# Yan-Xia/Text2Loc

Hardware: AMD Instinct MI355X
Metric: coarse-retrieval queries/sec over 11k-cell DB, embed_dim=256; top-1/3/5 recall parity (higher is better)
Workload: dtype f16; 1 GPU; KITTI360Pose-sized val DB: N=11259 cells x D=256 resident in HBM, Q=4096 precomputed text embeddings per step, top-10 (float64-exact ids); n_cells=11259, embed_dim=256, top_k=10, parallelism=single-gpu, layout=one resident DB, two launches per step (scan, re-rank)

## Files before the change

### text2loc_amd/csrc/capi.hip

```cpp
#include <limits.h>
#include <string.h>

#include "t2l_internal.h"

namespace t2l {

int fail(t2l_ctx* ctx, int code, const std::string& msg) {
  if (ctx) ctx->err = msg;
  return code;
}

void event_begin(t2l_ctx* ctx, const char* name, hipStream_t s) {
  if (!ctx->profile_events) return;
  EventRing& e = ctx->events[name];
  if (e.a.empty()) {
    e.a.resize(kEventRing);
    e.b.resize(kEventRing);
    for (int i = 0; i < kEventRing; ++i) {
      (void)hipEventCreate(&e.a[i]);
      (void)hipEventCreate(&e.b[i]);
    }
  }
  e.open = (e.calls++ % ctx->profile_events) == 0;
  if (e.open) (void)hipEventRecord(e.a[e.head], s);
// ... 558 lines not shown
    if (!ctx->search_auto) {
      ctx->escalated = false;
      ctx->heavy = false;
      ctx->all_exact = false;
      ctx->merge_live = true;
      ctx->stat_seen = ctx->stat_seq;
    }
  } else if (!strcmp(name, "search_heavy")) {
    ctx->heavy = value != 0;
  } else if (!strcmp(name, "search_small")) {
    ctx->search_small = value != 0;
  } else if (!strcmp(name, "search_small_wgs")) {
    if (value < 0 || value > 256) return fail(ctx, T2L_EINVAL, "search_small_wgs: 0 (default by query count: 128 or 192) .. 256 workgroups per slice");
    ctx->search_small_wgs = (int)value;
  } else if (!strcmp(name, "search_xcd_qgroups")) {
    if (value != 1 && value != 2 && value != 4 && value != 8) return fail(ctx, T2L_EINVAL, "search_xcd_qgroups must be 1, 2, 4 or 8");
    ctx->xcd_qgroups = (int)value;
  } else if (!strcmp(name, "text_train_bf16")) {
    if (value != 1 && value != 2)
      return fail(ctx, T2L_EINVAL, "text_train_bf16: 2 (default: split-bf16, the f32-class arithmetic) or 1 (bf16 operands); the f32-MFMA "
                                   "form (0) was removed in round 5 — it measured slower than PyTorch's f32 step");
    ctx->text_train_bf16 = (int)value;
  } else if (!strcmp(name, "encoder_two_cells")) {
    ctx->encoder_two_cells = value != 0;
  } else if (!strcmp(name, "search_merge_lists")) {
    if (value != 0 && value != 1 && value != 2) return fail(ctx, T2L_EINVAL, "search_merge_lists: 0 (plain lists), 1 (merged records), 2 (default: by report card)");
    ctx->search_merge = (int)value;
    ctx->merge_live = true;
  } else if (!strcmp(name, "search_wide_repair")) {
    if (value < 0 || value > 1024) return fail(ctx, T2L_EINVAL, "search_wide_repair: 0 (off) .. 1024 rows");
    ctx->wide_repair = (int)value;
  } else if (!strcmp(name, "search_tile_sel")) {
    ctx->search_tile_sel = value != 0;
  } else if (!strcmp(name, "search_pair_ll")) {
    if (value != 5 && value != 6) return fail(ctx, T2L_EINVAL, "search_pair_ll must be 5 or 6");
    ctx->pair_ll = (int)value;
  } else if (!strcmp(name, "train_gemm_block")) {
    if (value != 0 && value != 32 && value != 64) return fail(ctx, T2L_EINVAL, "train_gemm_block must be 0 (auto), 32 or 64");
    ctx->train_gemm_block = (int)value;
  } else if (!strcmp(name, "train_bf16")) {
    if (value != 0 && value != 1 && value != 2) return fail(ctx, T2L_EINVAL, "train_bf16: 0 (f32 MFMA), 1 (bf16 operands) or 2 (split-bf16, three products)");
    ctx->train_bf16 = (int)value;
  } else if (!strcmp(name, "train_keep_adam_state")) {
    ctx->train_keep_adam = value != 0;
  } else if (!strcmp(name, "profile_rerank")) {
    ctx->profile_rerank = value != 0;
  } else if (!strcmp(name, "stats_reset")) {
    for (auto& kv : ctx->events) {
      kv.second.count = 0;
      kv.second.calls = 0;
      kv.second.open = false;
    }
    ctx->span_read = ctx->busy_read = ctx->span_seq;
  } else if (!strcmp(name, "search_lanes")) {
    if (value < 1 || value > t2l_ctx::kMaxLanes) return fail(ctx, T2L_EINVAL, "search_lanes must be 1..4");
    T2L_HIP(ctx, hipDeviceSynchronize());
    for (auto& L : ctx->lanes) L.pending = false;
    ctx->n_lanes = (int)value;
  } else if (!strcmp(name, "stream_min_rows")) {
    ctx->stream_min_rows = (int)value;
  } else if (!strcmp(name, "pointnet_pyg_self_loops")) {
    ctx->pn_self_loops = value != 0;
  } else if (!strcmp(name, "profile_events")) {
    if (value < 0) return fail(ctx, T2L_EINVAL, "profile_events must be >= 0");
    ctx->profile_events = (int)value;
    for (auto& kv : ctx->events) kv.second.calls = 0;
// ... 10 lines not shown
  const bool busy = !strcmp(name, "search_scan_busy");
  if (busy || !strcmp(name, "search_scan_span")) {
    unsigned& cursor = busy ? ctx->busy_read : ctx->span_read;
    if (!ctx->scan_span || ctx->span_seq == cursor) return T2L_OK;
    T2L_HIP(ctx, hipDeviceSynchronize());
    std::vector<unsigned long long> h((size_t)2 * kSpanWgs * kSpanRing);
    T2L_HIP(ctx, hipMemcpy(h.data(), ctx->scan_span, sizeof(unsigned long long) * h.size(), hipMemcpyDeviceToHost));
    const unsigned first = ctx->span_seq - cursor > (unsigned)kSpanRing ? ctx->span_seq - kSpanRing + 1 : cursor + 1;
    double sum = 0.0;
    int n = 0;
    const unsigned long long tmask = (1ull << 40) - 1;
    for (unsigned q = first; q <= ctx->span_seq; ++q) {
      const unsigned long long* e = &h[(size_t)2 * kSpanWgs * (q % kSpanRing)];
      const unsigned grid = ctx->span_grid[q % kSpanRing];
      if (!grid) continue;
      unsigned long long t_min = ~0ull, t_max = 0, total = 0;
      bool ok = true;
      for (unsigned w = 0; w < grid && ok; ++w) {
        const unsigned long long a = e[2 * w], b = e[2 * w + 1];
        ok = (a >> 40) == (q & 0xFFFFFFu) && (b >> 40) == (q & 0xFFFFFFu);
        t_min = std::min(t_min, a & tmask);
        t_max = std::max(t_max, b & tmask);
        total += ((b & tmask) - (a & tmask)) & tmask;
      }
      if (!ok) continue;
      sum += (busy ? (double)total / grid : (double)((t_max - t_min) & tmask)) * 1e-5;
      ++n;
    }
    cursor = ctx->span_seq;
    if (n) *out_avg_ms = (float)(sum / n);
    *out_count = n;
    return T2L_OK;
  }
  auto it = ctx->events.find(name);
  if (it == ctx->events.end() || it->second.count == 0) return T2L_OK;
  EventRing& e = it->second;
  double sum = 0.0;
  for (int i = 0; i < e.count; ++i) {
    const int slot = ((e.head - 1 - i) % kEventRing + kEventRing) % kEventRing;
    T2L_HIP(ctx, hipEventSynchronize(e.b[slot]));
    float ms = 0.f;
    T2L_HIP(ctx, hipEventElapsedTime(&ms, e.a[slot], e.b[slot]));
    sum += ms;
  }
  *out_avg_ms = (float)(sum / e.count);
  *out_count = e.count;
  e.count = 0;
  return T2L_OK;
}

}
```

### text2loc_amd/csrc/search.hip

```cpp
#include <float.h>
#include <limits.h>

#include <type_traits>

#include "t2l_internal.h"
#include "search_dev.h"

namespace t2l {

__device__ __forceinline__ void reset_counts(int32_t* fb_count, int32_t* fb_prev, int zero_counts, int tid) {
  if (zero_counts && tid < 16) {
    fb_count[64 + tid] = fb_prev[tid];
    fb_prev[tid] = 0;
  }
  if (!zero_counts && tid == 0) {
    fb_count[12] += fb_count[4];
    fb_count[4] = fb_count[6] = 0;
  }
}


__global__ __launch_bounds__(256) void split_db_kernel(const float* __restrict__ db, uint4* __restrict__ out, int rows) {
  const int gid = blockIdx.x * 256 + threadIdx.x;
  const int row = gid >> 5, c = gid & 31;
// ... 228 lines not shown
  }
  asm volatile("s_waitcnt vmcnt(0)" ::: "memory");

  {
    const int row0 = (sp + (nt - 1) * nsplit) * kTileRows + 4 * half;
    const int code0 = (nt - 1) << 4;
    const bool odd = nt & 1;
#pragma unroll
    for (int r = 0; r < 16; ++r) {
      const bool ok = row0 + (r & 3) + 8 * (r >> 2) < n_rows;
      const float s0 = odd ? accA0[r] : accB0[r], s1 = odd ? accA1[r] : accB1[r];
      ins_key<LL>(w.ls0, ok ? make_key(s0, mask, code0 + r) : T2L_NEG_INF);
      ins_key<LL>(w.ls1, ok ? make_key(s1, mask, code0 + r) : T2L_NEG_INF);
    }
  }
  const int part = 2 * sp + half, parts = 2 * nsplit;
  if (qrow0 < Q) {
    float4* out = reinterpret_cast<float4*>(cand + ((size_t)qrow0 * parts + part) * LL);
#pragma unroll
    for (int i = 0; i < LL / 4; ++i) out[i] = make_float4(w.ls0[4 * i], w.ls0[4 * i + 1], w.ls0[4 * i + 2], w.ls0[4 * i + 3]);
  }
  if (qrow1 < Q) {
    float4* out = reinterpret_cast<float4*>(cand + ((size_t)qrow1 * parts + part) * LL);
#pragma unroll
    for (int i = 0; i < LL / 4; ++i) out[i] = make_float4(w.ls1[4 * i], w.ls1[4 * i + 1], w.ls1[4 * i + 2], w.ls1[4 * i + 3]);
  }
}

template <int CTRL>
__device__ __forceinline__ float dpp_f(float v) {
  return __uint_as_float((unsigned)__builtin_amdgcn_update_dpp(0, (int)__float_as_uint(v), CTRL, 0xF, 0xF, true));
}

struct RerankArgs {
  const float* db;
  const float* q;
  int Q, K, parts, code_bits;
  const float* cand;
  int row_offset;
  float eps_rel;
  const float* db_norm_max;
  int half_mode;
  int32_t* out_idx;
  double* out_score;
  int32_t* flags;
  int32_t* fb_count;
  float eps_rel_probe, pinf;
  int n_rows, defer, stat_mode;
  int32_t* host_stat;
  int seq, wide_cap;
  int rec6;
};

constexpr int kMergedLL = 8;
#ifndef T2L_SEL_RD
#define T2L_SEL_RD 2
#endif
template <int LL, int NS, bool MERGE = false, int SEL = 0>
__global__ __launch_bounds__(512, 1) void scanp_kernel(const uint4* __restrict__ dbt, int n_rows, int n_tiles, int code_bits,
                                                       const float* __restrict__ q, int Q, int nsplit,
                                                       float* __restrict__ cand, int32_t* __restrict__ fb_count, int32_t* __restrict__ fb_prev,
                                                       int zero_counts, float pinf, unsigned long long* __restrict__ span,
                                                       unsigned span_seq, int xcd_qgroups) {
  static_assert(NS == 4, "the step loop below is unrolled for a ring of 4 slots");
  static_assert(!MERGE || LL == 6, "the in-workgroup list merge is written for lists of 6");
  static_assert(!SEL || MERGE, "the tile-local selection's dropped-bound leaves through the merged record's bound");
  extern __shared__ __attribute__((aligned(16))) float smem[];
  constexpr int kSlotBytes = 2 * kHalfTileBytes;
  constexpr unsigned kExchange = 2 * kSlotBytes;
  const int tid = threadIdx.x, lane = tid & 63;
  const int half = lane >> 5, col = lane & 31;
  int sp = blockIdx.x % nsplit, qb = blockIdx.x / nsplit;
  if (xcd_qgroups > 1) {
    const int GQ = xcd_qgroups, GS = 8 / GQ, nqb = gridDim.x / nsplit;
    const int x = blockIdx.x & 7, j = blockIdx.x >> 3, per = nqb / GQ;
    qb = (j % per) * GQ + x % GQ;
    sp = (j / per) * GS + x / GQ;
  }
  const int uwave = uniform_wave_id();
  const int quad = uwave >> 2, wq = uwave & 3;
  const int vn = 2 * nsplit, vs = sp + quad * nsplit;
  const int nt = vs < n_tiles ? (n_tiles - vs + vn - 1) / vn : 0;
  const int steps = sp < n_tiles ? (n_tiles - sp + vn - 1) / vn : 0;
  constexpr int kCS = MERGE ? 2 : 0;
// ... 411 lines not shown
      const int b = __float_as_int(key), src = b & 3;
      return key_row(__int_as_float(b >> 2), 2 * (part + (src >> 1) * parts) + (src & 1), 2 * parts, code_bits, strided_rows);
    } else {
      return key_row(key, part, parts >> 1, code_bits, strided_rows);
    }
  };
  const float* __restrict__ cand = a.cand;
  const float eps_rel = a.eps_rel, eps_rel_probe = a.eps_rel_probe, pinf = a.pinf;
  const float* __restrict__ db_norm_max = a.db_norm_max;
  int32_t* __restrict__ out_idx = a.out_idx;
  double* __restrict__ out_score = a.out_score;
  int32_t* __restrict__ flags = a.flags;
  int32_t* __restrict__ fb_count = a.fb_count;
  const int n_rows = a.n_rows, defer = a.defer, wide_cap = a.wide_cap;

  float lst[LL];
  {
    const float* mine = cand + ((size_t)qid * parts + min(lane, parts - 1)) * LL;
    if constexpr (MG) {
      const float4 v0 = reinterpret_cast<const float4*>(mine)[0], v1 = reinterpret_cast<const float4*>(mine)[1];
      lst[0] = v0.x; lst[1] = v0.y; lst[2] = v0.z; lst[3] = v0.w;
      lst[4] = v1.x; lst[5] = v1.y; lst[6] = v1.z; lst[7] = v1.w;
    } else if constexpr (LL % 2 == 0) {
#pragma unroll
      for (int i = 0; i < LL / 2; ++i) {
        const float2 v = reinterpret_cast<const float2*>(mine)[i];
        lst[2 * i] = v.x;
        lst[2 * i + 1] = v.y;
      }
    } else {
#pragma unroll
      for (int i = 0; i < LL; ++i) lst[i] = mine[i];
    }
    if (lane >= parts) {
#pragma unroll
      for (int i = 0; i < LL; ++i) lst[i] = T2L_NEG_INF;
    }
  }
  const float lane_floor = lst[LL - 1];
  if constexpr (MG) lst[LL - 1] = T2L_NEG_INF;
  float b1 = T2L_NEG_INF;
  if constexpr (MG) {
    if (a.rec6) {
      b1 = lst[LL - 2];
      lst[LL - 2] = T2L_NEG_INF;
    }
  }
  const float floor_max = wave_max_f32(fmaxf(lane_floor, b1), pinf);
  const int seg = lane & 15;
  double qd[16];
  float q_absmax = 0.f;
  {
    const float4* qp = reinterpret_cast<const float4*>(q + (size_t)qid * kD) + seg;
#pragma unroll
    for (int i = 0; i < 4; ++i) {
      const float4 v = qp[16 * i];
      qd[4 * i] = (double)v.x;
      qd[4 * i + 1] = (double)v.y;
      qd[4 * i + 2] = (double)v.z;
      qd[4 * i + 3] = (double)v.w;
      q_absmax = fmaxf(fmaxf(fmaxf(q_absmax, fabsf(v.x)), fabsf(v.y)), fmaxf(fabsf(v.z), fabsf(v.w)));
    }
  }

  float my_key = T2L_NEG_INF;
  int my_part = 0;
  auto merge_round = [&](int r) {
    const float bk = wave_max_f32(lst[0], pinf);
    const unsigned long long who = __ballot(lst[0] == bk);
    const int bl = __ffsll((long long)who) - 1;
    if (lane == r) {
      my_key = bk;
      my_part = bl;
    }
    const bool pop = lane == bl;
#pragma unroll
    for (int i = 0; i < LL - 1; ++i) lst[i] = pop ? lst[i + 1] : lst[i];
    lst[LL - 1] = pop ? T2L_NEG_INF : lst[LL - 1];
  };
#pragma unroll
  for (int r = 0; r < L - 4; ++r) merge_round(r);
  int my_row = (lane < L - 4 && my_key != T2L_NEG_INF) ? krow(my_key, my_part) : INT_MAX;

  double kscale = 1.0;
  bool representable = true;
  {
    const float m = row16_max_f32(q_absmax);
    int sq, sd;
    representable = half_shift_of(m, sq);
    representable = half_shift_of(db_norm_max[1], sd) && representable;
    if (half_mode) {
      kscale = ldexp(1.0, -(sq + sd));
    } else {
      representable = representable && abs(sq - 14) <= 40 && abs(sd - 14) <= 40;
    }
  }

  double qn = 0.0;
#pragma unroll
  for (int i = 0; i < 16; ++i) qn += qd[i] * qd[i];
  qn = row16_sum_f64(qn);
  const double eps32 = (double)eps_rel * sqrt(qn) * (double)(*db_norm_max);
  constexpr int LA = L - 4;
  float4 rows[L / 4][4];
  auto gather = [&](int p) {
    const int row = __shfl(my_row, 4 * p + (lane >> 4));
#ifdef T2L_EXP_RERANK_TWICE
    {
      const int other = row == INT_MAX ? 0 : (row * 7 + 13) % n_rows;
      const float4* op = reinterpret_cast<const float4*>(db + (size_t)other * kD) + seg;
#pragma unroll
      for (int i = 0; i < 4; ++i) {
        float4 v = op[16 * i];
        asm volatile("" ::"v"(v.x), "v"(v.y), "v"(v.z), "v"(v.w));
      }
    }
#endif
    const float4* rp = reinterpret_cast<const float4*>(db + (size_t)(row == INT_MAX ? 0 : row) * kD) + seg;
#pragma unroll
    for (int i = 0; i < 4; ++i) rows[p][i] = rp[16 * i];
  };
  double my_d = -__builtin_inf();
  auto score = [&](int p) {
    double d0 = 0.0, d1 = 0.0;
#pragma unroll
    for (int i = 0; i < 4; ++i) {
      d0 += (double)rows[p][i].x * qd[4 * i];
      d1 += (double)rows[p][i].y * qd[4 * i + 1];
      d0 += (double)rows[p][i].z * qd[4 * i + 2];
      d1 += (double)rows[p][i].w * qd[4 * i + 3];
    }
    const double d = row16_sum_f64(d0 + d1);
    const double mine = __shfl(d, 16 * (lane & 3));
    if ((lane >> 2) == p && lane < L && my_row != INT_MAX) my_d = mine;
  };
  auto rank_among = [&](auto n_tag) {
    constexpr int N = decltype(n_tag)::value;
    int r = 0;
#pragma unroll
    for (int j = 0; j < N; ++j) {
      const unsigned long long bj = __double_as_longlong(my_d);
      const double dj = __longlong_as_double(((unsigned long long)__builtin_amdgcn_readlane((unsigned)(bj >> 32), j) << 32) |
                                             (unsigned)__builtin_amdgcn_readlane((unsigned)bj, j));
      const int ij = __builtin_amdgcn_readlane(my_row, j);
      r += (dj > my_d || (dj == my_d && ij < my_row)) ? 1 : 0;
    }
    return r;
  };
  auto emit = [&](bool ok, int r) {
    if (lane < K) {
      out_idx[(size_t)qid * K + lane] = -1;
      if (out_score) out_score[(size_t)qid * K + lane] = -__builtin_inf();
    }
    if (ok && r < K) {
      out_idx[(size_t)qid * K + r] = my_row + row_offset;
      if (out_score) out_score[(size_t)qid * K + r] = my_d;
    }
  };
#pragma unroll
  for (int p = 0; p < L / 4 - 1; ++p) gather(p);
#pragma unroll
  for (int p = 0; p < L / 4 - 1; ++p) score(p);
  bool early = false;
  if (K <= LA && representable && eps_rel_probe == 0.f) {
    const float gA = fmaxf(__uint_as_float(__builtin_amdgcn_readlane(__float_as_uint(my_key), LA - 1)), floor_max);
    if (gA != T2L_NEG_INF) {
      const int rA = rank_among(std::integral_constant<int, LA>{});
      const bool validA = lane < LA && my_row != INT_MAX;
      const unsigned long long kthA = __ballot(validA && rA == K - 1);
      if (kthA != 0ull) {
        const double dK = __shfl(my_d, __ffsll((long long)kthA) - 1);
        if (dK > (double)gA * kscale + key_slack(gA, slack_bits, eps32, kscale)) {
          emit(validA, rA);
          early = true;
        }
      }
    }
  }
  if (early) {
    if (lane == 0) flags[qid] = 0;
  } else {
#pragma unroll
  for (int r = L - 4; r < L; ++r) merge_round(r);
  if (lane >= L - 4 && lane < L && my_key != T2L_NEG_INF) my_row = krow(my_key, my_part);
  const float key_L = __uint_as_float(__builtin_amdgcn_readlane(__float_as_uint(my_key), L - 1));
  const float g = fmaxf(key_L, floor_max);
  gather(L / 4 - 1);
  bool fast_done = false;
  if constexpr (MG && L == 16) {
    int d_lane = -1;
    const float b1_max = a.rec6 ? wave_max_f32(b1, pinf) : T2L_NEG_INF;
    if (b1_max != T2L_NEG_INF && b1_max > fmaxf(key_L, wave_max_f32(lane_floor, pinf)) && representable && K <= LA && eps_rel_probe == 0.f) {
      const int rA = rank_among(std::integral_constant<int, LA>{});
      const unsigned long long kthA = __ballot(lane < LA && my_row != INT_MAX && rA == K - 1);
      if (kthA != 0ull) {
        const double dKA = __shfl(my_d, __ffsll((long long)kthA) - 1);
        const double tA = (dKA - 2.0 * (fabs(dKA) * ldexp(1.0, slack_bits - 22) + eps32)) / kscale;
        float thrA = (float)tA;
        if ((double)thrA > tA) thrA = __uint_as_float(__float_as_uint(thrA) + (thrA > 0.f ? -1 : 1));
        if (fabs(tA) < 3.0e38) {
          const unsigned long long bm = __ballot(lane_floor != T2L_NEG_INF && lane_floor >= thrA);
          const unsigned long long dm = __ballot(b1 != T2L_NEG_INF && b1 >= thrA);
          if (bm == 0ull && __popcll(dm) == 1) d_lane = __ffsll((long long)dm) - 1;
        }
      }
    }
    if (d_lane >= 0) {
      const int kb = __shfl(__float_as_int(b1), d_lane);
      int cand_row = INT_MAX;
      if (lane >= L && lane < L + kTileSelGroup) {
        const int r = krow(__int_as_float((kb & ~((kTileSelGroup - 1) << 2)) | ((lane - L) << 2)), d_lane);
        cand_row = r < n_rows ? r : INT_MAX;
      }
#pragma unroll
      for (int j = 0; j < L; ++j) cand_row = __builtin_amdgcn_readlane(my_row, j) == cand_row ? INT_MAX : cand_row;
      if (lane >= L && lane < L + kTileSelGroup) my_row = cand_row;
      auto gather_d = [&](int p, float4 (&rw)[4]) {
        const int row = __shfl(my_row, L + 4 * p + (lane >> 4));
        const float4* rp = reinterpret_cast<const float4*>(db + (size_t)(row == INT_MAX ? 0 : row) * kD) + seg;
#pragma unroll
        for (int i = 0; i < 4; ++i) rw[i] = rp[16 * i];
      };
      auto score_d = [&](int p, const float4 (&rw)[4]) {
        double d0 = 0.0, d1 = 0.0;
#pragma unroll
        for (int i = 0; i < 4; ++i) {
          d0 += (double)rw[i].x * qd[4 * i];
          d1 += (double)rw[i].y * qd[4 * i + 1];
          d0 += (double)rw[i].z * qd[4 * i + 2];
          d1 += (double)rw[i].w * qd[4 * i + 3];
        }
        const double d = row16_sum_f64(d0 + d1);
        const double mine = __shfl(d, 16 * (lane & 3));
        if ((lane >> 2) == L / 4 + p && my_row != INT_MAX) my_d = mine;
      };
      static_assert(kTileSelGroup == 8, "two row groups of four");
      gather_d(0, rows[0]);
      gather_d(1, rows[1]);
      score(L / 4 - 1);
      score_d(0, rows[0]);
      score_d(1, rows[1]);
      const int rank2 = rank_among(std::integral_constant<int, L + kTileSelGroup>{});
      const bool valid2 = lane < L + kTileSelGroup && my_row != INT_MAX;
      const unsigned long long kth2 = __ballot(valid2 && rank2 == K - 1);
      const float g2 = fmaxf(key_L, wave_max_f32(lane == d_lane ? lane_floor : fmaxf(lane_floor, b1), pinf));
      if (kth2 != 0ull) {
        const double dK2 = __shfl(my_d, __ffsll((long long)kth2) - 1);
        if (dK2 > (double)g2 * kscale + key_slack(g2, slack_bits, eps32, kscale)) {
          emit(valid2, rank2);
          if (lane == 0) {
            flags[qid] = 0;
            atomicAdd(&fb_count[1], 1);
          }
          fast_done = true;
        }
      }
      if (!fast_done && lane >= L) {
        my_row = INT_MAX;
        my_d = -__builtin_inf();
      }
    } else {
      score(L / 4 - 1);
    }
  } else {
    score(L / 4 - 1);
  }
  if (!fast_done) {
  const int rank = rank_among(std::integral_constant<int, L>{});
  const bool valid = lane < L && my_row != INT_MAX;
  emit(valid, rank);

  bool certified = true;
  float thr = T2L_NEG_INF;
  if (g != T2L_NEG_INF) {
    certified = false;
    const unsigned long long kth = __ballot(valid && rank == K - 1);
    if (K <= L && kth != 0ull) {
      const double dK = __shfl(my_d, __ffsll((long long)kth) - 1);
      certified = dK > (double)g * kscale + key_slack(g, slack_bits, eps32, kscale);
      if (eps_rel_probe > 0.f && lane == 0 &&
          !(dK > (double)g * kscale + key_slack(g, slack_bits, (double)eps_rel_probe * sqrt(qn) * (double)(*db_norm_max), kscale)))
        atomicAdd(&fb_count[3], 1);
      const double S = 2.0 * (fabs(dK) * ldexp(1.0, slack_bits - 22) + eps32);
      const double t = (dK - S) / kscale;
      thr = (float)t;
      if ((double)thr > t) thr = __uint_as_float(__float_as_uint(thr) + (thr > 0.f ? -1 : 1));
      if (!(fabs(t) < 3.0e38)) thr = T2L_NEG_INF;
    }
  }
  bool settled = false;
  if (!certified && representable && thr != T2L_NEG_INF && L + 16 <= 64) {
    int cnt = 0;
#pragma unroll
    for (int i = 0; i < LL; ++i) cnt += (lst[i] >= thr) ? 1 : 0;
    int total = cnt;
#pragma unroll
    for (int off = 32; off >= 1; off >>= 1) total += __shfl_xor(total, off);
    bool bad = lane_floor != T2L_NEG_INF && lane_floor >= thr;
// ... 13 lines not shown
#pragma unroll
          for (int i = 0; i < LL - 1; ++i) lst[i] = lst[i + 1];
          lst[LL - 1] = T2L_NEG_INF;
        }
      }
      int n_ent = L + total;
      if constexpr (MG) {
        for (unsigned long long m = d_mask; m != 0ull; m &= m - 1ull) {
          const int b = __ffsll((long long)m) - 1;
          const int kb = __shfl(__float_as_int(b1), b);
          int cand_row = INT_MAX;
          if (lane < kTileSelGroup) {
            const int r = krow(__int_as_float((kb & ~((kTileSelGroup - 1) << 2)) | (lane << 2)), b);
            cand_row = r < n_rows ? r : INT_MAX;
          }
          bool dup = cand_row == INT_MAX;
          for (int j = 0; j < n_ent; ++j) dup = dup || __builtin_amdgcn_readlane(my_row, j) == cand_row;
          const unsigned long long keep = __ballot(!dup);
          if (!dup) wr_buf[__popcll(keep & ((1ull << lane) - 1ull))] = cand_row;
          __builtin_amdgcn_fence(__ATOMIC_SEQ_CST, "workgroup");
          const int nk = __popcll(keep);
          if (lane >= n_ent && lane < n_ent + nk) my_row = wr_buf[lane - n_ent];
          __builtin_amdgcn_fence(__ATOMIC_SEQ_CST, "workgroup");
          n_ent += nk;
        }
      }
      for (int p = L / 4; p < (n_ent + 3) / 4; ++p) {
        const int row = __shfl(my_row, 4 * p + (lane >> 4));
        const float4* rp = reinterpret_cast<const float4*>(db + (size_t)(row == INT_MAX ? 0 : row) * kD) + seg;
        double d0 = 0.0, d1 = 0.0;
#pragma unroll
        for (int i = 0; i < 4; ++i) {
          const float4 rv = rp[16 * i];
          d0 += (double)rv.x * qd[4 * i];
          d1 += (double)rv.y * qd[4 * i + 1];
          d0 += (double)rv.z * qd[4 * i + 2];
          d1 += (double)rv.w * qd[4 * i + 3];
        }
        const double d = row16_sum_f64(d0 + d1);
        const double mine = __shfl(d, 16 * (lane & 3));
        if ((lane >> 2) == p && lane < n_ent && my_row != INT_MAX) my_d = mine;
      }
      int rank2 = 0;
      for (int j = 0; j < n_ent; ++j) {
        const unsigned long long bj = __double_as_longlong(my_d);
        const double dj = __longlong_as_double(((unsigned long long)__builtin_amdgcn_readlane((unsigned)(bj >> 32), j) << 32) |
                                               (unsigned)__builtin_amdgcn_readlane((unsigned)bj, j));
        const int ij = __builtin_amdgcn_readlane(my_row, j);
        rank2 += (dj > my_d || (dj == my_d && ij < my_row)) ? 1 : 0;
      }
      if (lane < n_ent && my_row != INT_MAX && rank2 < K) {
        out_idx[(size_t)qid * K + rank2] = my_row + row_offset;
        if (out_score) out_score[(size_t)qid * K + rank2] = my_d;
      }
      settled = true;
    } else {
      const int vn_ = MG ? 2 * parts : parts >> 1;
      constexpr int kRowsPerTile = MG ? 64 : 16;
      const int n_tiles_ = (n_rows + kTileRows - 1) / kTileRows;
      const int my_vs = MG ? lane : lane >> 1;
      const int my_nt = (lane < parts && my_vs < n_tiles_) ? (n_tiles_ - my_vs + vn_ - 1) / vn_ : 0;
      int work = bad ? my_nt * kRowsPerTile : cnt + (dbad ? kTileSelGroup : 0);
#pragma unroll
      for (int off = 32; off >= 1; off >>= 1) work += __shfl_xor(work, off);
      if (work <= wide_cap) {
        int* wr = wr_buf;
        const unsigned long long lt_mask = (1ull << lane) - 1ull;
        int base = 0;
#pragma unroll
        for (int i = 0; i < LL; ++i) {
// ... 22 lines not shown
          }
          base += nb;
        }
        __builtin_amdgcn_fence(__ATOMIC_SEQ_CST, "workgroup");
        double ts = -__builtin_inf();
        int tr = INT_MAX;
        for (int j = 0; j < L; ++j) {
          const double cd = __shfl(my_d, j);
          const int cr = __shfl(my_row, j);
          if (cr != INT_MAX) top32_insert(ts, tr, cd, cr, lane);
        }
        const int n_round = (base + 3) >> 2;
        auto row_of = [&](int p) {
          const int i = 4 * p + (lane >> 4);
          return i < base ? wr[i] : INT_MAX;
        };
        float4 cur[4], nxt[4];
        int row_c = n_round > 0 ? row_of(0) : INT_MAX, row_n = INT_MAX;
        {
          const float4* rp = reinterpret_cast<const float4*>(db + (size_t)(row_c == INT_MAX ? 0 : row_c) * kD) + seg;
#pragma unroll
          for (int i = 0; i < 4; ++i) cur[i] = rp[16 * i];
        }
        for (int p = 0; p < n_round; ++p) {
          if (p + 1 < n_round) {
            row_n = row_of(p + 1);
            const float4* rp = reinterpret_cast<const float4*>(db + (size_t)(row_n == INT_MAX ? 0 : row_n) * kD) + seg;
#pragma unroll
            for (int i = 0; i < 4; ++i) nxt[i] = rp[16 * i];
          }
          double d0 = 0.0, d1 = 0.0;
#pragma unroll
          for (int i = 0; i < 4; ++i) {
            d0 += (double)cur[i].x * qd[4 * i];
            d1 += (double)cur[i].y * qd[4 * i + 1];
            d0 += (double)cur[i].z * qd[4 * i + 2];
            d1 += (double)cur[i].w * qd[4 * i + 3];
          }
          const double d = row16_sum_f64(d0 + d1);
#pragma unroll
          for (int c = 0; c < 4; ++c) {
            const double cd = __shfl(d, 16 * c);
            const int cr = __shfl(row_c, 16 * c);
            if (cr != INT_MAX) top32_insert(ts, tr, cd, cr, lane);
          }
#pragma unroll
          for (int i = 0; i < 4; ++i) cur[i] = nxt[i];
          row_c = row_n;
        }
        if (lane < K) {
          out_idx[(size_t)qid * K + lane] = tr == INT_MAX ? -1 : tr + row_offset;
          if (out_score) out_score[(size_t)qid * K + lane] = ts;
        }
        if (lane == 0) atomicAdd(&fb_count[5], 1);
        settled = true;
      }
    }
  }
  if (lane == 0) {
    const int flag = !representable ? 2 : ((certified || settled) ? 0 : 1);
    flags[qid] = flag;
    if (!certified || !representable) atomicAdd(&fb_count[1], 1);
    if (flag) {
      atomicAdd(&fb_count[2], 1);
      if (!defer) *my_wg_flag = flag;
      else if (flag == 2) flags[4 * Q + atomicAdd(&fb_count[6], 1)] = qid;
      else flags[3 * Q + atomicAdd(&fb_count[4], 1)] = qid;
    }
  }
  }
  }
}

template <int LL, int L, bool MG = false>
__global__ __launch_bounds__(256, (MG ? 4 : 1)) void rerank_kernel(const float* __restrict__ db, const float* __restrict__ q, int Q,
                                                     int K, int parts, int code_bits,
                                                     const float* __restrict__ cand, int row_offset, float eps_rel,
                                                     const float* __restrict__ db_norm_max, int half_mode,
                                                     int32_t* __restrict__ out_idx, double* __restrict__ out_score,
                                                     int32_t* __restrict__ flags, int32_t* __restrict__ fb_count,
                                                     float eps_rel_probe, float pinf, int n_rows, int defer, int stat_mode,
                                                     int32_t* __restrict__ host_stat, int seq, int wide_cap, int rec6) {
  __shared__ WgExactShared exact_sh;
  __shared__ int wg_flag[4];
  __shared__ int wide_rows[4][kWideCap];
  const RerankArgs a{db, q, Q, K, parts, code_bits, cand, row_offset, eps_rel, db_norm_max, half_mode, out_idx, out_score, flags, fb_count,
                     eps_rel_probe, pinf, n_rows, defer, stat_mode, host_stat, seq, wide_cap, rec6};
  const int lane = threadIdx.x & 63;
  const int qid = blockIdx.x * 4 + (threadIdx.x >> 6);
  if (threadIdx.x < 4) wg_flag[threadIdx.x] = 0;
  if (blockIdx.x == 0 && threadIdx.x == 0) publish_report(a);
  __syncthreads();
  if (qid < Q) rerank_query<LL, L, MG>(a, qid, lane, &wg_flag[threadIdx.x >> 6], wide_rows[threadIdx.x >> 6]);
  __syncthreads();
#pragma unroll 1
  for (int w = 0; w < 4; ++w) {
    if (!wg_flag[w]) continue;
    const int fq = blockIdx.x * 4 + w;
    if (threadIdx.x == 0) atomicAdd(&fb_count[0], 1);
    wg_exact_scan(db, n_rows, q + (size_t)fq * kD, K, row_offset, out_idx + (size_t)fq * K,
                  out_score ? out_score + (size_t)fq * K : nullptr, exact_sh);
  }
}

__global__ __launch_bounds__(256) void db_norm_kernel(const float* __restrict__ db, int n_rows, float* out) {
  __shared__ float red[4];
  __shared__ int red_a[4];
  const int lane = threadIdx.x & 63, wave = threadIdx.x >> 6;
  float m = 0.f;
  int am = 0;
  for (int row = blockIdx.x * 4 + wave; row < n_rows; row += gridDim.x * 4) {
    const float4 v = reinterpret_cast<const float4*>(db + (size_t)row * kD)[lane];
    float s = v.x * v.x + v.y * v.y + v.z * v.z + v.w * v.w;
    int a = max(max(__float_as_int(v.x) & 0x7fffffff, __float_as_int(v.y) & 0x7fffffff),
                max(__float_as_int(v.z) & 0x7fffffff, __float_as_int(v.w) & 0x7fffffff));
#pragma unroll
    for (int off = 32; off >= 1; off >>= 1) {
      s += __shfl_xor(s, off);
      a = max(a, __shfl_xor(a, off));
    }
// ... 131 lines not shown
  event_begin(ctx, "search_scan", s);
  if (ctx->eff_mode == 0) {
    const dim3 grid((Q + kWideQPerBlock - 1) / kWideQPerBlock * nsplit);
    const size_t lds = (size_t)4 * kHalfTileBytes;
    static PerDeviceOnce once;
    if (once.need(ctx->device)) {
      allow_lds(&scanh_kernel<LL>, (size_t)4 * kHalfTileBytes);
      once.mark(ctx->device);
    }
    hipLaunchKernelGGL((scanh_kernel<LL>), grid, dim3(256), lds, s, dbh, n_rows, n_tiles, code_bits, q, Q, nsplit,
                       ctx->cand_score, ctx->fb_count, ctx->fb_prev, zero, __builtin_inff());
  } else if (ctx->eff_mode == 2) {
    const dim3 grid((Q + kWideQPerBlock - 1) / kWideQPerBlock * nsplit);
    const size_t lds = (size_t)4 * kTileFloats * sizeof(float);
    static PerDeviceOnce once;
    if (once.need(ctx->device)) {
      allow_lds(&scanw_kernel<LL, 4>, (size_t)4 * kTileFloats * sizeof(float));
      once.mark(ctx->device);
    }
    hipLaunchKernelGGL((scanw_kernel<LL, 4>), grid, dim3(256), lds, s, dbs, n_rows, n_tiles, code_bits, q, Q, nsplit,
                       ctx->cand_score, ctx->fb_count, ctx->fb_prev, zero, __builtin_inff());
  }
  event_end(ctx, "search_scan", s);
  }
  T2L_HIP(ctx, hipGetLastError());
  hipEvent_t ea, eb;
  if constexpr (LL == 6 && L == 16) {
    if (merged) {
      const bool evr = ctx->profile_rerank && event_pair(ctx, "search_rerank", &ea, &eb);
      if (evr)
        hipExtLaunchKernelGGL((rerank_kernel<kMergedLL, L, true>), dim3((Q + 3) / 4), dim3(256), 0u, s, ea, eb, 0u, db, q, Q, K, nsplit / 2,
                              code_bits, (const float*)ctx->cand_score, row_offset, eps_rel, (const float*)ctx->db_norm_max, half_mode, out_idx,
                              out_score, ctx->flags, ctx->fb_count, eps_probe, __builtin_inff(), n_rows, defer, stat_mode,
                              ctx->host_stat_dev, seq, min(ctx->wide_repair, kWideCap), ctx->search_tile_sel ? 1 : 0);
      else
        hipLaunchKernelGGL((rerank_kernel<kMergedLL, L, true>), dim3((Q + 3) / 4), dim3(256), 0, s, db, q, Q, K, nsplit / 2, code_bits,
                           ctx->cand_score, row_offset, eps_rel, ctx->db_norm_max, half_mode, out_idx, out_score, ctx->flags,
                           ctx->fb_count, eps_probe, __builtin_inff(), n_rows, defer, stat_mode, ctx->host_stat_dev, seq,
                           min(ctx->wide_repair, kWideCap), ctx->search_tile_sel ? 1 : 0);
      T2L_HIP(ctx, hipGetLastError());
      if (ctx->heavy) return exact_stage_impl(ctx, db, n_rows, row_offset, q, Q, K, out_idx, out_score, s);
      return T2L_OK;
    }
  }
  if (ctx->profile_rerank && event_pair(ctx, "search_rerank", &ea, &eb))
    hipExtLaunchKernelGGL((rerank_kernel<LL, L>), dim3((Q + 3) / 4), dim3(256), 0u, s, ea, eb, 0u, db, q, Q, K, parts, code_bits,
                          (const float*)ctx->cand_score, row_offset, eps_rel, (const float*)ctx->db_norm_max, half_mode, out_idx,
                          out_score, ctx->flags, ctx->fb_count, eps_probe, __builtin_inff(), n_rows, defer, stat_mode,
                          ctx->host_stat_dev, seq, min(ctx->wide_repair, kWideCap), 0);
  else
    hipLaunchKernelGGL((rerank_kernel<LL, L>), dim3((Q + 3) / 4), dim3(256), 0, s, db, q, Q, K, parts, code_bits,
                       ctx->cand_score, row_offset, eps_rel, ctx->db_norm_max, half_mode, out_idx, out_score, ctx->flags,
                       ctx->fb_count, eps_probe, __builtin_inff(), n_rows, defer, stat_mode, ctx->host_stat_dev, seq,
                       min(ctx->wide_repair, kWideCap), 0);
  T2L_HIP(ctx, hipGetLastError());
  if (ctx->heavy) return exact_stage_impl(ctx, db, n_rows, row_offset, q, Q, K, out_idx, out_score, s);
  return T2L_OK;
}


__global__ __launch_bounds__(256) void empty_result_kernel(int n, int32_t* __restrict__ out_idx, double* __restrict__ out_score) {
  const int i = blockIdx.x * 256 + threadIdx.x;
  if (i < n) {
    out_idx[i] = -1;
    if (out_score) out_score[i] = -__builtin_inf();
  }
}

__global__ __launch_bounds__(256) void all_exact_prep_kernel(int Q, int32_t* __restrict__ list, int32_t* __restrict__ fb_count,
                                                             int32_t* __restrict__ fb_prev, int32_t* __restrict__ host_stat, int seq) {
  if (blockIdx.x == 0) {
    reset_counts(fb_count, fb_prev, 1, threadIdx.x);
    __syncthreads();
    if (threadIdx.x == 0) {
      if (host_stat && seq > 0) {
        host_stat[1] = fb_count[64 + 10] == 2 ? fb_count[64 + 3] : fb_count[64 + 2];
        host_stat[2] = fb_count[64 + 9];
        host_stat[3] = fb_count[64 + 0] + fb_count[64 + 4] + fb_count[64 + 12];
        host_stat[4] = fb_count[64 + 10];
        host_stat[5] = fb_count[64 + 10] == 2 ? fb_count[64 + 3] : fb_count[64 + 1];
        __hip_atomic_store(&host_stat[0], seq, __ATOMIC_RELEASE, __HIP_MEMORY_SCOPE_SYSTEM);
      }
      fb_count[9] = Q;
      fb_count[10] = 0;
      fb_count[1] = fb_count[2] = fb_count[4] = Q;
    }
  }
// ... 174 lines not shown
```

### text2loc_amd/csrc/t2l_internal.h

```cpp
#pragma once
#include <hip/hip_runtime.h>

#include <atomic>
#include <hip/hip_ext.h>
#include <stdint.h>

#include <string>
#include <unordered_map>
#include <vector>

#include "t2l.h"

namespace t2l {

constexpr int kD = T2L_EMBED_DIM;
constexpr int kS = T2L_OBJECT_SIZE;
constexpr int kSP = 32;

constexpr int kTileRows = 32;
constexpr int kRowStrideF = kD + 4;
constexpr int kTileFloats = kTileRows * kRowStrideF;
constexpr int kQPerWave = 32;
constexpr int kScanWaves = 4;
constexpr int kQPerBlock = kQPerWave * kScanWaves;
// ... 39 lines not shown
  int32_t* fb_count = nullptr;
  int32_t* fb_prev = nullptr;
  int32_t* seg_idx = nullptr;
  double* seg_score = nullptr;
  size_t cand_cap = 0, flag_cap = 0, seg_idx_cap = 0, seg_score_cap = 0;
  void* loss_ws = nullptr;
  size_t loss_ws_cap = 0;
  void* reduce_ws = nullptr;
  size_t reduce_ws_cap = 0;
  t2l::EncoderWeights* enc = nullptr;
  void* train = nullptr;
  void* pn = nullptr;
  void* fine = nullptr;
  void* fine_train = nullptr;
  void* text_head = nullptr;
  void* text_train = nullptr;
  int (*sync_fn)(void* user, double* buf, int64_t n, void* stream) = nullptr;
  void* sync_user = nullptr;
  double* sync_buf = nullptr;
  bool sync_failed = false;
  void* fast_ws = nullptr;
  size_t fast_ws_cap = 0;
  float* fast_zero = nullptr;
  int text_head_rows = 0;
  int pn_self_loops = 1;
  double eps_scale = 1.0;
  int nsplit_override = 0;
  int search_mode = 0;
  int encoder_f32 = 0;
  int encoder_f16 = 0;
  int search_auto = 1;
  int pair_ll = 6;
  int search_tile_sel = 1;
  int search_small = 1;
  int search_small_wgs = 0;
  bool last_search_small = false;
  unsigned* small_ticket = nullptr;
  unsigned small_ticket_base[4] = {0, 0, 0, 0};
  void* small_part = nullptr;
  size_t small_part_cap = 0;
  int wide_repair = 512;
  int encoder_two_cells = 1;
  int search_merge = 2;
  bool merge_live = true;
  int xcd_qgroups = 4;
  int train_bf16 = 0;
  int text_train_bf16 = 2;
  int train_gemm_block = 0;
  int train_keep_adam = 0;
  int eff_mode = 0;
  bool heavy = false;
  bool all_exact = false;
  unsigned all_exact_calls = 0;
  bool escalated = false;
  int32_t* host_stat = nullptr;
  int32_t* host_stat_dev = nullptr;
  int stat_seq = 0, stat_seen = 0;
  struct SearchLane {
    float* cand_score = nullptr;
    size_t cand_cap = 0, flag_cap = 0;
    int32_t *flags = nullptr, *fb_count = nullptr, *fb_prev = nullptr, *host_stat = nullptr, *host_stat_dev = nullptr;
    int stat_seen = 0;
    hipStream_t stream = nullptr;
    hipEvent_t done = nullptr;
    bool pending = false, ready = false;
  };
// ... 115 lines not shown
```

Before: 102.1 million queries/s.

## Add predicted early gather of the last rerank slot and trim query registers

Adds an opt-in predictor in the rerank kernel that decides before scoring whether the last candidate group will be needed. If so, it merges and issues that gather early to overlap its latency with scoring. The query is now held as f32 float4 registers and converted to double at use instead of a 16-entry double array, which lowers register pressure. The -1 prefill of outputs is skipped when every result lane is valid. Optional device counters and a query API report how often the prediction fires.

Result: no change. 101.4 million queries/s (-0.7%).

```diff
diff --git a/text2loc_amd/csrc/capi.hip b/text2loc_amd/csrc/capi.hip
--- a/text2loc_amd/csrc/capi.hip
+++ b/text2loc_amd/csrc/capi.hip
@@ -614,6 +614,11 @@
     ctx->wide_repair = (int)value;
   } else if (!strcmp(name, "search_tile_sel")) {
     ctx->search_tile_sel = value != 0;
+  } else if (!strcmp(name, "search_rerank_predict")) {
+    if (value != 0 && value != 1) return fail(ctx, T2L_EINVAL, "search_rerank_predict must be 0 or 1");
+    ctx->search_rerank_predict = (int)value;
+  } else if (!strcmp(name, "search_rerank_count")) {
+    ctx->search_rerank_count = value != 0;
   } else if (!strcmp(name, "search_pair_ll")) {
     if (value != 5 && value != 6) return fail(ctx, T2L_EINVAL, "search_pair_ll must be 5 or 6");
     ctx->pair_ll = (int)value;
@@ -690,6 +695,15 @@
     *out_count = n;
     return T2L_OK;
   }
+  const bool late = !strcmp(name, "search_rerank_predicted_late");
+  if (late || !strcmp(name, "search_rerank_second_trips")) {
+    int32_t c = 0;
+    T2L_HIP(ctx, hipSetDevice(ctx->device));
+    T2L_HIP(ctx, hipDeviceSynchronize());
+    if (!ctx->last_search_small) T2L_HIP(ctx, hipMemcpy(&c, ctx->fb_count + (late ? 13 : 14), sizeof(c), hipMemcpyDeviceToHost));
+    *out_count = c;
+    return T2L_OK;
+  }
   auto it = ctx->events.find(name);
   if (it == ctx->events.end() || it->second.count == 0) return T2L_OK;
   EventRing& e = it->second;
diff --git a/text2loc_amd/csrc/search.hip b/text2loc_amd/csrc/search.hip
--- a/text2loc_amd/csrc/search.hip
+++ b/text2loc_amd/csrc/search.hip
@@ -284,6 +284,11 @@
   return __uint_as_float((unsigned)__builtin_amdgcn_update_dpp(0, (int)__float_as_uint(v), CTRL, 0xF, 0xF, true));
 }
 
+#ifndef T2L_RERANK_PREDICT_M4
+#define T2L_RERANK_PREDICT_M4 2
+#endif
+constexpr int kPredictM4 = T2L_RERANK_PREDICT_M4;
+
 struct RerankArgs {
   const float* db;
   const float* q;
@@ -302,6 +307,7 @@
   int32_t* host_stat;
   int seq, wide_cap;
   int rec6;
+  int predict;
 };
 
 constexpr int kMergedLL = 8;
@@ -779,6 +785,15 @@
 #pragma unroll
       for (int i = 0; i < LL; ++i) lst[i] = mine[i];
     }
+  }
+  const int seg = lane & 15;
+  float4 qv[4];
+  {
+    const float4* qp = reinterpret_cast<const float4*>(q + (size_t)qid * kD) + seg;
+#pragma unroll
+    for (int i = 0; i < 4; ++i) qv[i] = qp[16 * i];
+  }
+  {
     if (lane >= parts) {
 #pragma unroll
       for (int i = 0; i < LL; ++i) lst[i] = T2L_NEG_INF;
@@ -794,18 +809,16 @@
     }
   }
   const float floor_max = wave_max_f32(fmaxf(lane_floor, b1), pinf);
-  const int seg = lane & 15;
-  double qd[16];
+  auto qd = [&](int i, int c) -> double {
+    float x = c == 0 ? qv[i].x : c == 1 ? qv[i].y : c == 2 ? qv[i].z : qv[i].w;
+    if constexpr (L == 16) asm volatile("" : "+v"(x));
+    return (double)x;
+  };
   float q_absmax = 0.f;
   {
-    const float4* qp = reinterpret_cast<const float4*>(q + (size_t)qid * kD) + seg;
 #pragma unroll
     for (int i = 0; i < 4; ++i) {
-      const float4 v = qp[16 * i];
-      qd[4 * i] = (double)v.x;
-      qd[4 * i + 1] = (double)v.y;
-      qd[4 * i + 2] = (double)v.z;
-      qd[4 * i + 3] = (double)v.w;
+      const float4 v = qv[i];
       q_absmax = fmaxf(fmaxf(fmaxf(q_absmax, fabsf(v.x)), fabsf(v.y)), fmaxf(fabsf(v.z), fabsf(v.w)));
     }
   }
@@ -845,12 +858,17 @@
 
   double qn = 0.0;
 #pragma unroll
-  for (int i = 0; i < 16; ++i) qn += qd[i] * qd[i];
+  for (int i = 0; i < 16; ++i) {
+    const double x = qd(i >> 2, i & 3);
+    qn += x * x;
+  }
   qn = row16_sum_f64(qn);
   const double eps32 = (double)eps_rel * sqrt(qn) * (double)(*db_norm_max);
   constexpr int LA = L - 4;
+  constexpr bool kPredict = L == 16 && LL <= 8;
+  constexpr int kLastSlot = L / 4 - 1;
   float4 rows[L / 4][4];
-  auto gather = [&](int p) {
+  auto gather = [&](int p, int slot) {
     const int row = __shfl(my_row, 4 * p + (lane >> 4));
 #ifdef T2L_EXP_RERANK_TWICE
     {
@@ -865,17 +883,17 @@
 #endif
     const float4* rp = reinterpret_cast<const float4*>(db + (size_t)(row == INT_MAX ? 0 : row) * kD) + seg;
 #pragma unroll
-    for (int i = 0; i < 4; ++i) rows[p][i] = rp[16 * i];
+    for (int i = 0; i < 4; ++i) rows[slot][i] = rp[16 * i];
   };
   double my_d = -__builtin_inf();
-  auto score = [&](int p) {
+  auto score = [&](int p, int slot) {
     double d0 = 0.0, d1 = 0.0;
 #pragma unroll
     for (int i = 0; i < 4; ++i) {
-      d0 += (double)rows[p][i].x * qd[4 * i];
-      d1 += (double)rows[p][i].y * qd[4 * i + 1];
-      d0 += (double)rows[p][i].z * qd[4 * i + 2];
-      d1 += (double)rows[p][i].w * qd[4 * i + 3];
+      d0 += (double)rows[slot][i].x * qd(i, 0);
+      d1 += (double)rows[slot][i].y * qd(i, 1);
+      d0 += (double)rows[slot][i].z * qd(i, 2);
+      d1 += (double)rows[slot][i].w * qd(i, 3);
     }
     const double d = row16_sum_f64(d0 + d1);
     const double mine = __shfl(d, 16 * (lane & 3));
@@ -895,7 +913,8 @@
     return r;
   };
   auto emit = [&](bool ok, int r) {
-    if (lane < K) {
+    const bool full = representable && __popcll(__ballot(ok && r < K)) == K;
+    if (!full && lane < K) {
       out_idx[(size_t)qid * K + lane] = -1;
       if (out_score) out_score[(size_t)qid * K + lane] = -__builtin_inf();
     }
@@ -905,9 +924,27 @@
     }
   };
 #pragma unroll
-  for (int p = 0; p < L / 4 - 1; ++p) gather(p);
-#pragma unroll
-  for (int p = 0; p < L / 4 - 1; ++p) score(p);
+  for (int p = 0; p < L / 4 - 1; ++p) gather(p, p);
+  bool late = false;
+  if constexpr (kPredict) {
+    if ((a.predict & 1) && K <= LA && representable && eps_rel_probe == 0.f) {
+      const float gA = fmaxf(__uint_as_float(__builtin_amdgcn_readlane(__float_as_uint(my_key), LA - 1)), floor_max);
+      const float kK = __uint_as_float(__builtin_amdgcn_readlane(__float_as_uint(my_key), K - 1));
+      if (gA != T2L_NEG_INF) {
+        late = !((double)kK * kscale - (kPredictM4 * 0.25) * key_slack(kK, slack_bits, eps32, kscale) >
+                 (double)gA * kscale + key_slack(gA, slack_bits, eps32, kscale));
+        if (late) {
+#pragma unroll
+          for (int r = L - 4; r < L; ++r) merge_round(r);
+          if (lane >= L - 4 && lane < L && my_key != T2L_NEG_INF) my_row = krow(my_key, my_part);
+          gather(L / 4 - 1, kLastSlot);
+          if (lane == 0 && (a.predict & 2)) atomicAdd(&fb_count[13], 1);
+        }
+      }
+    }
+  }
+#pragma unroll
+  for (int p = 0; p < L / 4 - 1; ++p) score(p, p);
   bool early = false;
   if (K <= LA && representable && eps_rel_probe == 0.f) {
     const float gA = fmaxf(__uint_as_float(__builtin_amdgcn_readlane(__float_as_uint(my_key), LA - 1)), floor_max);
@@ -927,12 +964,17 @@
   if (early) {
     if (lane == 0) flags[qid] = 0;
   } else {
-#pragma unroll
-  for (int r = L - 4; r < L; ++r) merge_round(r);
-  if (lane >= L - 4 && lane < L && my_key != T2L_NEG_INF) my_row = krow(my_key, my_part);
+  if (!late) {
+#pragma unroll
+    for (int r = L - 4; r < L; ++r) merge_round(r);
+    if (lane >= L - 4 && lane < L && my_key != T2L_NEG_INF) my_row = krow(my_key, my_part);
+  }
   const float key_L = __uint_as_float(__builtin_amdgcn_readlane(__float_as_uint(my_key), L - 1));
   const float g = fmaxf(key_L, floor_max);
-  gather(L / 4 - 1);
+  if (!late) {
+    gather(L / 4 - 1, kLastSlot);
+    if (lane == 0 && (a.predict & 2) && K <= LA && representable && eps_rel_probe == 0.f) atomicAdd(&fb_count[14], 1);
+  }
   bool fast_done = false;
   if constexpr (MG && L == 16) {
     int d_lane = -1;
@@ -972,10 +1014,10 @@
         double d0 = 0.0, d1 = 0.0;
 #pragma unroll
         for (int i = 0; i < 4; ++i) {
-          d0 += (double)rw[i].x * qd[4 * i];
-          d1 += (double)rw[i].y * qd[4 * i + 1];
-          d0 += (double)rw[i].z * qd[4 * i + 2];
-          d1 += (double)rw[i].w * qd[4 * i + 3];
+          d0 += (double)rw[i].x * qd(i, 0);
+          d1 += (double)rw[i].y * qd(i, 1);
+          d0 += (double)rw[i].z * qd(i, 2);
+          d1 += (double)rw[i].w * qd(i, 3);
         }
         const double d = row16_sum_f64(d0 + d1);
         const double mine = __shfl(d, 16 * (lane & 3));
@@ -984,7 +1026,8 @@
       static_assert(kTileSelGroup == 8, "two row groups of four");
       gather_d(0, rows[0]);
       gather_d(1, rows[1]);
-      score(L / 4 - 1);
+      if (late && lane == 0 && (a.predict & 2)) atomicAdd(&fb_count[14], 1);
+      score(L / 4 - 1, kLastSlot);
       score_d(0, rows[0]);
       score_d(1, rows[1]);
       const int rank2 = rank_among(std::integral_constant<int, L + kTileSelGroup>{});
@@ -1007,10 +1050,10 @@
         my_d = -__builtin_inf();
       }
     } else {
-      score(L / 4 - 1);
+      score(L / 4 - 1, kLastSlot);
     }
   } else {
-    score(L / 4 - 1);
+    score(L / 4 - 1, kLastSlot);
   }
   if (!fast_done) {
   const int rank = rank_among(std::integral_constant<int, L>{});
@@ -1090,10 +1133,10 @@
 #pragma unroll
         for (int i = 0; i < 4; ++i) {
           const float4 rv = rp[16 * i];
-          d0 += (double)rv.x * qd[4 * i];
-          d1 += (double)rv.y * qd[4 * i + 1];
-          d0 += (double)rv.z * qd[4 * i + 2];
-          d1 += (double)rv.w * qd[4 * i + 3];
+          d0 += (double)rv.x * qd(i, 0);
+          d1 += (double)rv.y * qd(i, 1);
+          d0 += (double)rv.z * qd(i, 2);
+          d1 += (double)rv.w * qd(i, 3);
         }
         const double d = row16_sum_f64(d0 + d1);
         const double mine = __shfl(d, 16 * (lane & 3));
@@ -1182,10 +1225,10 @@
           double d0 = 0.0, d1 = 0.0;
 #pragma unroll
           for (int i = 0; i < 4; ++i) {
-            d0 += (double)cur[i].x * qd[4 * i];
-            d1 += (double)cur[i].y * qd[4 * i + 1];
-            d0 += (double)cur[i].z * qd[4 * i + 2];
-            d1 += (double)cur[i].w * qd[4 * i + 3];
+            d0 += (double)cur[i].x * qd(i, 0);
+            d1 += (double)cur[i].y * qd(i, 1);
+            d0 += (double)cur[i].z * qd(i, 2);
+            d1 += (double)cur[i].w * qd(i, 3);
           }
           const double d = row16_sum_f64(d0 + d1);
 #pragma unroll
@@ -1230,12 +1273,12 @@
                                                      int32_t* __restrict__ out_idx, double* __restrict__ out_score,
                                                      int32_t* __restrict__ flags, int32_t* __restrict__ fb_count,
                                                      float eps_rel_probe, float pinf, int n_rows, int defer, int stat_mode,
-                                                     int32_t* __restrict__ host_stat, int seq, int wide_cap, int rec6) {
+                                                     int32_t* __restrict__ host_stat, int seq, int wide_cap, int rec6, int predict) {
   __shared__ WgExactShared exact_sh;
   __shared__ int wg_flag[4];
   __shared__ int wide_rows[4][kWideCap];
   const RerankArgs a{db, q, Q, K, parts, code_bits, cand, row_offset, eps_rel, db_norm_max, half_mode, out_idx, out_score, flags, fb_count,
-                     eps_rel_probe, pinf, n_rows, defer, stat_mode, host_stat, seq, wide_cap, rec6};
+                     eps_rel_probe, pinf, n_rows, defer, stat_mode, host_stat, seq, wide_cap, rec6, predict};
   const int lane = threadIdx.x & 63;
   const int qid = blockIdx.x * 4 + (threadIdx.x >> 6);
   if (threadIdx.x < 4) wg_flag[threadIdx.x] = 0;
@@ -1433,12 +1476,12 @@
         hipExtLaunchKernelGGL((rerank_kernel<kMergedLL, L, true>), dim3((Q + 3) / 4), dim3(256), 0u, s, ea, eb, 0u, db, q, Q, K, nsplit / 2,
                               code_bits, (const float*)ctx->cand_score, row_offset, eps_rel, (const float*)ctx->db_norm_max, half_mode, out_idx,
                               out_score, ctx->flags, ctx->fb_count, eps_probe, __builtin_inff(), n_rows, defer, stat_mode,
-                              ctx->host_stat_dev, seq, min(ctx->wide_repair, kWideCap), ctx->search_tile_sel ? 1 : 0);
+                              ctx->host_stat_dev, seq, min(ctx->wide_repair, kWideCap), ctx->search_tile_sel ? 1 : 0, ctx->search_rerank_predict | (ctx->search_rerank_count << 1));
       else
         hipLaunchKernelGGL((rerank_kernel<kMergedLL, L, true>), dim3((Q + 3) / 4), dim3(256), 0, s, db, q, Q, K, nsplit / 2, code_bits,
                            ctx->cand_score, row_offset, eps_rel, ctx->db_norm_max, half_mode, out_idx, out_score, ctx->flags,
                            ctx->fb_count, eps_probe, __builtin_inff(), n_rows, defer, stat_mode, ctx->host_stat_dev, seq,
-                           min(ctx->wide_repair, kWideCap), ctx->search_tile_sel ? 1 : 0);
+                           min(ctx->wide_repair, kWideCap), ctx->search_tile_sel ? 1 : 0, ctx->search_rerank_predict | (ctx->search_rerank_count << 1));
       T2L_HIP(ctx, hipGetLastError());
       if (ctx->heavy) return exact_stage_impl(ctx, db, n_rows, row_offset, q, Q, K, out_idx, out_score, s);
       return T2L_OK;
@@ -1448,12 +1491,12 @@
     hipExtLaunchKernelGGL((rerank_kernel<LL, L>), dim3((Q + 3) / 4), dim3(256), 0u, s, ea, eb, 0u, db, q, Q, K, parts, code_bits,
                           (const float*)ctx->cand_score, row_offset, eps_rel, (const float*)ctx->db_norm_max, half_mode, out_idx,
                           out_score, ctx->flags, ctx->fb_count, eps_probe, __builtin_inff(), n_rows, defer, stat_mode,
-                          ctx->host_stat_dev, seq, min(ctx->wide_repair, kWideCap), 0);
+                          ctx->host_stat_dev, seq, min(ctx->wide_repair, kWideCap), 0, ctx->search_rerank_predict | (ctx->search_rerank_count << 1));
   else
     hipLaunchKernelGGL((rerank_kernel<LL, L>), dim3((Q + 3) / 4), dim3(256), 0, s, db, q, Q, K, parts, code_bits,
                        ctx->cand_score, row_offset, eps_rel, ctx->db_norm_max, half_mode, out_idx, out_score, ctx->flags,
                        ctx->fb_count, eps_probe, __builtin_inff(), n_rows, defer, stat_mode, ctx->host_stat_dev, seq,
-                       min(ctx->wide_repair, kWideCap), 0);
+                       min(ctx->wide_repair, kWideCap), 0, ctx->search_rerank_predict | (ctx->search_rerank_count << 1));
   T2L_HIP(ctx, hipGetLastError());
   if (ctx->heavy) return exact_stage_impl(ctx, db, n_rows, row_offset, q, Q, K, out_idx, out_score, s);
   return T2L_OK;
diff --git a/text2loc_amd/csrc/t2l_internal.h b/text2loc_amd/csrc/t2l_internal.h
--- a/text2loc_amd/csrc/t2l_internal.h
+++ b/text2loc_amd/csrc/t2l_internal.h
@@ -95,6 +95,8 @@
   int search_auto = 1;
   int pair_ll = 6;
   int search_tile_sel = 1;
+  int search_rerank_predict = 0;
+  int search_rerank_count = 0;
   int search_small = 1;
   int search_small_wgs = 0;
   bool last_search_small = false;
```
